# adwardlee/RenderIH

Measured on AMD Instinct MI355X. Metric: images/sec fwd+bwd @256x256 two-hand, higher is better.
Workload: dtype f32; 1 GPU; BASELINE configs[1]: batch=64/GPU 256x256 ResNet50 + cross-hand attention decoder, fwd + loss + bwd + Adam step, dropout 0.05, fp32; global_batch=64, parallelism=dp1, hipgraph=True, backward_stages=1, weight_gradients_on_side_stream=False, grad_allreduce=none (1 rank), optimizer=renderih_amd.optim.Adam (rih_adam_multi, one launch), flash_attention=True, one_kernel_attention_rih_fused_attn=False

## Files before the change

### include/renderih_amd.h

```cpp
#ifndef RENDERIH_AMD_H
#define RENDERIH_AMD_H

#include <stdint.h>

#ifdef __cplusplus
extern "C" {
#endif

#define RIH_OK 0
#define RIH_EINVAL (-1)

typedef struct rih_gemm_desc {
    const float* A;
    const float* B;
    float* C;
    const float* bias;
    const float* R;
    int32_t M, N, K;
    int32_t lda, ldb, ldc, ldr;
    int32_t a_mode, b_mode;
    int32_t nb1, nb2;
    int64_t sA1, sA2, sB1, sB2, sC1, sC2;
    int32_t splitk;
    int32_t kchunk;
// ... 46 lines not shown
    float* dst;
    float* db;
    int32_t S, Mp, M, N, Cin, taps, CinValid, accumulate;
    int32_t CinPitch;
    int32_t reserved;
} rih_reduce_desc;
int rih_splitk_reduce_multi(const rih_reduce_desc* descs, int n, void* stream);
int rih_splitk_reduce_bias_batched(const float* P, int S, int Mp, int M, int N, float* dst, int Cin, int taps,
                                   int CinValid, int accumulate, float* db, int nb, int64_t sP, int64_t sDst,
                                   int64_t sDb, void* stream);

int rih_bn_stats_from_blocks(const float* part, int T, int C, int rows, int rows_per_block, float eps, float momentum,
                             float* mean, float* invstd, float* running_mean, float* running_var, void* stream);

typedef struct rih_conv3_desc {
    const float* x;
    const void* w_h2;
    float* y;
    float* stats;
    const float* amax_x;
    const float* amax_w;
    int32_t imgs, H, W, C, N, ldx, ldy, Kpad, relu;
    int32_t ldr;
    const float* r;
} rih_conv3_desc;
int rih_conv3x3_ok(const rih_conv3_desc* d);
int rih_conv3x3_stats_rows(const rih_conv3_desc* d);
int rih_conv3x3(const rih_conv3_desc* d, void* stream);
typedef struct rih_h2_desc {
    const float* w;
    void* dst;
    const float* amax;
    int32_t Cout, Cin, KH, KW, CinPad, for_dgrad, Kpad;
} rih_h2_desc;
int rih_h2_multi(const rih_h2_desc* descs, int n, void* stream);

typedef struct rih_panel_desc {
    const float* a;
    const void* w_h2;
    float* c;
    const float* r;
    float* stats;
    const float* amax_a;
    const float* amax_w;
    int32_t M, N, K, lda, ldc, ldr, relu;
} rih_panel_desc;
int rih_panel_ok(const rih_panel_desc* d);
int rih_panel_stats_rows(const rih_panel_desc* d);
int rih_panel(const rih_panel_desc* d, void* stream);
int rih_stem_ok(const rih_conv3_desc* d);
int rih_stem(const rih_conv3_desc* d, void* stream);
int rih_rows_ok(const rih_panel_desc* d);
int rih_rows_stats_rows(const rih_panel_desc* d);
int rih_rows(const rih_panel_desc* d, void* stream);
int rih_rows_tile(const rih_panel_desc* d, int* bm, int* bn);
int rih_rows_tiled(const rih_panel_desc* d, int bm, int bn, void* stream);

int rih_splitk_finish(const float* P, int S, int M, int N, float* C, int ldc, const float* bias, const float* R,
                      int ldr, float alpha, int relu, void* stream);

int rih_pack_conv_weight(const float* w, float* dst, int Cout, int Cin, int KH, int KW, int CinPad,
                         int for_dgrad, void* stream);
typedef struct rih_pack_desc {
    const float* w;
    float* dst;
    int32_t Cout, Cin, KH, KW, CinPad, mode, kh0, kw0, step, Th, Tw, reserved;
} rih_pack_desc;
int rih_pack_conv_weight_multi(const rih_pack_desc* descs, int n, void* stream);
int rih_pack_conv_weight_sub(const float* w, float* dst, int Cout, int Cin, int KH, int KW, int CinPad, int kh0,
                             int kw0, int step, int Th, int Tw, void* stream);

int rih_nchw_to_nhwc(const float* x, float* y, int N, int C, int H, int W, int Cpad, void* stream);
int rih_nhwc_to_nchw(const float* x, float* y, int N, int C, int H, int W, int ldx, void* stream);
int rih_maxpool3x3s2_fwd(const float* x, float* y, int8_t* arg, int N, int H, int W, int C, void* stream);
int rih_maxpool3x3s2_bwd(const float* dy, const int8_t* arg, float* dx, int N, int H, int W, int C, void* stream);
int rih_avgpool_fwd(const float* x, float* y, int N, int HW, int C, void* stream);
int rih_avgpool_bwd(const float* dy, float* dx, int N, int HW, int C, void* stream);
int rih_upsample2x_fwd(const float* x, float* y, int N, int H, int W, int C, void* stream);
int rih_upsample2x_bwd(const float* dy, float* dx, int N, int H, int W, int C, void* stream);
int rih_upsample_bilinear_fwd(const float* x, float* y, int N, int H, int W, int C, int factor, void* stream);
int rih_upsample_bilinear_bwd(const float* dy, float* dx, int N, int H, int W, int C, int factor, void* stream);
int rih_nearest_up_add_fwd(const float* x, const float* add, float* y, int N, int H, int W, int C, int factor,
                           void* stream);
int rih_nearest_up_bwd(const float* dy, float* dx, int N, int H, int W, int C, int factor, void* stream);

int64_t rih_bn_ws_floats(int rows, int C);
int rih_bn_stats(const float* x, int rows, int C, float eps, float momentum, float* mean, float* invstd,
                 float* running_mean, float* running_var, float* ws, void* stream);
int rih_bn_eval_stats(const float* running_mean, const float* running_var, int C, float eps, float* mean,
                      float* invstd, void* stream);
int rih_bn_apply(const float* x, const float* mean, const float* invstd, const float* gamma, const float* beta,
                 const float* residual, float* y, int rows, int C, int relu, uint8_t* relu_mask, float* amax, void* stream);
int rih_bn_bwd(const float* dy, const float* x, const float* y, const float* mean, const float* invstd,
               const float* gamma, float* dx, float* dres, float* dgamma, float* dbeta, int rows, int C,
               int relu, int frozen_stats, float* ws, const uint8_t* relu_mask, float* amax_dx, void* stream);

int rih_layernorm_fwd(const float* x, const float* x2, const float* g, const float* b, float* y, float* mean,
                      float* rstd, int rows, int D, float eps, int relu, void* stream);
int rih_ln_nblk(int rows);
// ... 265 lines not shown
```

### renderih_amd/_lib.py

```python
import ctypes as C
import os

from . import _build

c_f = C.c_void_p
c_i = C.c_int
c_l = C.c_int64
c_u64 = C.c_uint64
c_fl = C.c_float


class GemmDesc(C.Structure):
    _fields_ = [('A', C.c_void_p), ('B', C.c_void_p), ('C', C.c_void_p), ('bias', C.c_void_p), ('R', C.c_void_p),
                ('M', C.c_int32), ('N', C.c_int32), ('K', C.c_int32),
                ('lda', C.c_int32), ('ldb', C.c_int32), ('ldc', C.c_int32), ('ldr', C.c_int32),
                ('a_mode', C.c_int32), ('b_mode', C.c_int32),
                ('nb1', C.c_int32), ('nb2', C.c_int32),
                ('sA1', C.c_int64), ('sA2', C.c_int64), ('sB1', C.c_int64), ('sB2', C.c_int64),
                ('sC1', C.c_int64), ('sC2', C.c_int64),
                ('splitk', C.c_int32), ('kchunk', C.c_int32), ('sCsplit', C.c_int64),
                ('alpha', C.c_float), ('relu', C.c_int32),
                ('H', C.c_int32), ('W', C.c_int32), ('Cin', C.c_int32), ('Ho', C.c_int32), ('Wo', C.c_int32),
                ('KH', C.c_int32), ('KW', C.c_int32), ('strideA', C.c_int32), ('upS', C.c_int32),
                ('padH', C.c_int32), ('padW', C.c_int32), ('tile', C.c_int32), ('engine', C.c_int32),
                ('cS', C.c_int32), ('cOH', C.c_int32), ('cOW', C.c_int32), ('cH', C.c_int32), ('cW', C.c_int32), ('ones_row', C.c_int32),
                ('reserved0', C.c_int32), ('sBias1', C.c_int64), ('sR1', C.c_int64), ('stats', C.c_void_p),
                ('drop_p', C.c_float), ('reserved1', C.c_int32), ('drop_seed', C.c_uint64), ('drop_seed_dev', C.c_void_p),
                ('amax_a', C.c_void_p), ('amax_b', C.c_void_p),
                ('a_seg', C.c_void_p * 3), ('lda_seg', C.c_int32 * 3), ('k_seg', C.c_int32 * 3)]


class ReduceDesc(C.Structure):
    _fields_ = [('P', C.c_void_p), ('dst', C.c_void_p), ('db', C.c_void_p)] + \
               [(n, C.c_int32) for n in ('S', 'Mp', 'M', 'N', 'Cin', 'taps', 'CinValid', 'accumulate', 'CinPitch', 'reserved')]


class Conv3Desc(C.Structure):
    _fields_ = [('x', C.c_void_p), ('w_h2', C.c_void_p), ('y', C.c_void_p), ('stats', C.c_void_p), ('amax_x', C.c_void_p),
                ('amax_w', C.c_void_p)] + \
               [(n, C.c_int32) for n in ('imgs', 'H', 'W', 'C', 'N', 'ldx', 'ldy', 'Kpad', 'relu', 'ldr')] + [('r', C.c_void_p)]


class PanelDesc(C.Structure):
    _fields_ = [('a', C.c_void_p), ('w_h2', C.c_void_p), ('c', C.c_void_p), ('r', C.c_void_p), ('stats', C.c_void_p),
                ('amax_a', C.c_void_p), ('amax_w', C.c_void_p)] + \
               [(n, C.c_int32) for n in ('M', 'N', 'K', 'lda', 'ldc', 'ldr', 'relu')]


class H2Desc(C.Structure):
    _fields_ = [('w', C.c_void_p), ('dst', C.c_void_p), ('amax', C.c_void_p)] + \
               [(n, C.c_int32) for n in ('Cout', 'Cin', 'KH', 'KW', 'CinPad', 'for_dgrad', 'Kpad')]


class AbsmaxDesc(C.Structure):
    _fields_ = [('x', C.c_void_p), ('out', C.c_void_p), ('n', C.c_int64)]


BOUND_FLOATS = 2048


class LnFinalDesc(C.Structure):
    _fields_ = [('ws', C.c_void_p), ('dg', C.c_void_p), ('db', C.c_void_p), ('D', C.c_int32), ('nblk', C.c_int32)]


class PackDesc(C.Structure):
    _fields_ = [('w', C.c_void_p), ('dst', C.c_void_p)] + \
               [(n, C.c_int32) for n in ('Cout', 'Cin', 'KH', 'KW', 'CinPad', 'mode', 'kh0', 'kw0', 'step', 'Th', 'Tw',
                                         'reserved')]


class HConvDesc(C.Structure):
    _fields_ = [('x', C.c_void_p), ('w', C.c_void_p), ('zero', C.c_void_p), ('bias', C.c_void_p),
                ('post_scale', C.c_void_p), ('post_shift', C.c_void_p), ('res', C.c_void_p), ('y', C.c_void_p)] + \
               [(n, C.c_int32) for n in ('N', 'H', 'W', 'Cin', 'Cout', 'KH', 'KW', 'stride', 'pad', 'Ho', 'Wo',
                                         'ldx', 'ldr', 'ldy', 'Kpad', 'relu', 'out_f32')]


class ManoModel(C.Structure):
    _fields_ = [('comps', C.c_void_p), ('hands_mean', C.c_void_p), ('shapedirs', C.c_void_p),
                ('posedirs', C.c_void_p), ('v_template', C.c_void_p), ('J_reg', C.c_void_p),
                ('weights', C.c_void_p), ('parent', C.c_int32 * 16)]


class MeshTopo(C.Structure):
# ... 220 lines not shown
```

### renderih_amd/csrc/rih_conv3.hip

```cpp
#include <hip/hip_runtime.h>
#include <stdint.h>
#include <stdlib.h>
#include "../../include/renderih_amd.h"
#include "rih_e2.h"

typedef float floatx16 __attribute__((ext_vector_type(16)));
typedef _Float16 f16x8 __attribute__((ext_vector_type(8)));

namespace {

constexpr int A_STAGE = 340 * 128;
constexpr int NT = 512;

struct C3Args {
    const float* x;
    const unsigned char* w;
    float* y;
    float* stats;
    const float* amax_x;
    const float* amax_w;
    int imgs, H, W, C, N, ldx, ldy, Kp, relu;
    int tiles_x, tiles_y, nblk;
    const float* r;
    int ldr;
// ... 204 lines not shown
                const int row = (lane >> 3) + 8 * q, c4 = (lane & 7) * 4;
                const int ty = (TW == 32) ? blk : 2 * blk + (row >> 4), tx = row & (TW - 1);
                float4 v = *reinterpret_cast<const float4*>(stg + row * SLD + c4);
                if (RES) {
                    const float4 rr = *reinterpret_cast<const float4*>(rpatch + ((long long)ty * p.W + tx) * p.ldr + j * 32 + c4);
                    v.x += rr.x; v.y += rr.y; v.z += rr.z; v.w += rr.w;
                }
                if (p.relu) { v.x = fmaxf(v.x, 0.f); v.y = fmaxf(v.y, 0.f); v.z = fmaxf(v.z, 0.f); v.w = fmaxf(v.w, 0.f); }
                *reinterpret_cast<float4*>(ypatch + ((long long)ty * p.W + tx) * p.ldy + j * 32 + c4) = v;
                if (STATS) RIH_E2_STATS_ADD(j, v)
            }
        }
    }
    if (STATS) {
        const long long rb = (((long long)img * p.tiles_y + ty_t) * p.tiles_x + tx_t) * WGM + wm;
#pragma unroll
        for (int j = 0; j < TN; ++j) {
            RIH_E2_STATS_MERGE(j, mean, m2)
            if ((lane >> 3) == 0) {
                const int nn = n0 + wn * (BN / WGN) + j * 32 + (lane & 7) * 4;
                *reinterpret_cast<float4*>(p.stats + (rb * 2 + 0) * p.N + nn) = mean;
                *reinterpret_cast<float4*>(p.stats + (rb * 2 + 1) * p.N + nn) = m2;
            }
        }
    }
}

struct H2WArgs {
    const float* w;
    unsigned char* dst;
    const float* amax;
    int N, K, Kp, for_dgrad;
    int Cout, Cin, KH, KW, CinPad;
};
__device__ __forceinline__ float h2w_fetch(const H2WArgs& a, int n, int k) {
    if (k >= a.K) return 0.f;
    if (!a.for_dgrad) {
        const int tap = k / a.CinPad, ci = k - tap * a.CinPad;
        return ci < a.Cin ? a.w[((long long)n * a.Cin + ci) * (a.KH * a.KW) + tap] : 0.f;
    }
    const int co = k % a.Cout, t = k / a.Cout;
    const int tw = t % a.KW, th = t / a.KW;
    const int kh = a.KH - 1 - th, kw = a.KW - 1 - tw;
    return n < a.Cin ? a.w[(((long long)co * a.Cin + n) * a.KH + kh) * a.KW + kw] : 0.f;
}
__device__ __forceinline__ void h2w_span(const H2WArgs& a, long long first, long long stride) {
    const int G = a.Kp / 8;
    const long long total = (long long)a.N * G;
    const float sc = e2_scale(a.amax);
    for (long long i = first; i < total; i += stride) {
        const int n = (int)(i / G), g = (int)(i - (long long)n * G);
        uint4 h, l;
        e2_split2h(h2w_fetch(a, n, 8 * g + 0), h2w_fetch(a, n, 8 * g + 1), sc, h.x, l.x);
        e2_split2h(h2w_fetch(a, n, 8 * g + 2), h2w_fetch(a, n, 8 * g + 3), sc, h.y, l.y);
        e2_split2h(h2w_fetch(a, n, 8 * g + 4), h2w_fetch(a, n, 8 * g + 5), sc, h.z, l.z);
        e2_split2h(h2w_fetch(a, n, 8 * g + 6), h2w_fetch(a, n, 8 * g + 7), sc, h.w, l.w);
        uint4* d = reinterpret_cast<uint4*>(a.dst + i * 32);
        d[0] = h;
        d[1] = l;
    }
}
constexpr int H2_PACK = 48;
struct H2Pack {
    H2WArgs d[H2_PACK];
    int first[H2_PACK + 1];
    int n;
};
static_assert(sizeof(H2Pack) <= 4096, "kernel argument limit");
__global__ __launch_bounds__(256) void h2_weight_multi_kernel(const H2Pack pk) {
    const int b = (int)blockIdx.x;
    int k = 0;
    while (k + 1 < pk.n && b >= pk.first[k + 1]) ++k;
    const int nb = pk.first[k + 1] - pk.first[k];
    h2w_span(pk.d[k], (long long)(b - pk.first[k]) * 256 + threadIdx.x, (long long)nb * 256);
}

int h2_args(H2WArgs& a, const rih_h2_desc& d) {
    if (!d.w || !d.dst || !d.amax || d.Cout < 1 || d.Cin < 1 || d.KH < 1 || d.KW < 1 || d.CinPad < d.Cin || d.Kpad < 32 ||
        d.Kpad % 32 != 0 || ((uintptr_t)d.dst % 16) != 0)
        return RIH_EINVAL;
    a.w = d.w; a.dst = (unsigned char*)d.dst; a.amax = d.amax; a.Kp = d.Kpad; a.for_dgrad = d.for_dgrad ? 1 : 0;
    a.Cout = d.Cout; a.Cin = d.Cin; a.KH = d.KH; a.KW = d.KW; a.CinPad = d.CinPad;
    if (!a.for_dgrad) { a.N = d.Cout; a.K = d.KH * d.KW * d.CinPad; }
    else { a.N = d.CinPad; a.K = d.KH * d.KW * d.Cout; }
    return a.Kp < a.K ? RIH_EINVAL : RIH_OK;
}


struct PanelArgs {
    const float* a;
    const unsigned char* w;
    float* c;
    const float* r;
    float* stats;
    const float* amax_a;
    const float* amax_w;
    int M, N, K, lda, ldc, ldr, relu;
    int nblk, mtiles;
};

template <int KT, int BN, bool STATS, bool RES>
__global__ __launch_bounds__(NT, 2) void panel_kernel(const PanelArgs p) {
    constexpr int K = 32 * KT;
    constexpr int BM = 8192 / K;
    constexpr int WGN = BN >= 128 ? 4 : 2, WGM = 8 / WGN;
    constexpr int TM = BM / WGM / 32, TN = BN / WGN / 32;
    static_assert(TM >= 1 && TN >= 1 && BN * K <= 16384, "tile shape");
    constexpr int ROWB = K * 4;
    constexpr int UPR = K / 4;
    constexpr int A_ST = BM * ROWB;
    constexpr int B_BYTES = BN * ROWB;
    constexpr int NPA = (BM * K / 4) / NT;
    constexpr int NPB = (BN * UPR) / NT;
    static_assert((BM * K / 4) % NT == 0 && (BN * UPR) % NT == 0 && 8 * 32 * 32 * 4 <= A_ST, "loader / staging geometry");
    __shared__ __attribute__((aligned(16))) unsigned char smem[B_BYTES + 2 * A_ST];
    unsigned char* const Bs = smem;
    unsigned char* const Abuf = smem + B_BYTES;
// ... 574 lines not shown
    rows_tile(d, bm, bn);
    return rih_rows_tiled(d, bm, bn, stream);
}

extern "C" int rih_stem_ok(const rih_conv3_desc* d) { return stem_ok(d) ? 1 : 0; }

extern "C" int rih_stem(const rih_conv3_desc* d, void* stream) {
    if (!stem_ok(d)) return RIH_EINVAL;
    RowsArgs a;
    a.a = d->x; a.w = (const unsigned char*)d->w_h2; a.c = d->y; a.r = nullptr; a.stats = d->stats;
    a.amax_a = d->amax_x; a.amax_w = d->amax_w;
    a.H = d->H; a.W = d->W; a.Ho = d->H / 2; a.Wo = d->W / 2;
    a.M = d->imgs * a.Ho * a.Wo; a.N = d->N; a.K = d->Kpad; a.lda = 4; a.ldc = d->ldy; a.ldr = 0; a.relu = d->relu ? 1 : 0;
    a.nblk = 1;
    a.mtiles = a.M / 256;
    hipStream_t s = (hipStream_t)stream;
    if (d->stats != nullptr) hipLaunchKernelGGL((rows_kernel<256, 64, true, false, true>), dim3((unsigned)a.mtiles), dim3(NT), 0, s, a);
    else hipLaunchKernelGGL((rows_kernel<256, 64, false, false, true>), dim3((unsigned)a.mtiles), dim3(NT), 0, s, a);
    return (int)hipGetLastError();
}

extern "C" int rih_h2_multi(const rih_h2_desc* descs, int n, void* stream) {
    if (n < 0 || (n > 0 && !descs)) return RIH_EINVAL;
    for (int i0 = 0; i0 < n; i0 += H2_PACK) {
        H2Pack pk;
        pk.n = (n - i0 < H2_PACK) ? n - i0 : H2_PACK;
        int total = 0;
        for (int i = 0; i < pk.n; ++i) {
            const int rc = h2_args(pk.d[i], descs[i0 + i]);
            if (rc != RIH_OK) return rc;
            const long long units = (long long)pk.d[i].N * (pk.d[i].Kp / 8);
            long long nb = (units + 255) / 256;
            if (nb > 512) nb = 512;
            pk.first[i] = total;
            total += (int)nb;
        }
        pk.first[pk.n] = total;
        hipLaunchKernelGGL(h2_weight_multi_kernel, dim3(total), dim3(256), 0, (hipStream_t)stream, pk);
    }
    return (int)hipGetLastError();
}
```

### renderih_amd/csrc/rih_gemm.hip

```cpp
#include <hip/hip_runtime.h>
#include <stdint.h>
#include <stdlib.h>
#include "../../include/renderih_amd.h"
#include "rih_hash.h"
#include "rih_e2.h"

typedef float floatx16 __attribute__((ext_vector_type(16)));
typedef __bf16 bf16x8 __attribute__((ext_vector_type(8)));
typedef __bf16 bf16x2 __attribute__((ext_vector_type(2)));
typedef _Float16 f16x8 __attribute__((ext_vector_type(8)));

namespace {

constexpr int BK = 32;

struct GemmArgs {
    const float* A;
    const float* B;
    float* C;
    const float* bias;
    const float* R;
    int M, N, K;
    int lda, ldb, ldc, ldr;
    int nb2, splitk, kchunk;
// ... 1071 lines not shown
    __shared__ float tile[8][33];
    const int tx = threadIdx.x & 31, ty = threadIdx.x >> 5;
    const int tilesN = (N + 31) / 32;
    const int m0 = (bx / tilesN) * 8, n0 = (bx % tilesN) * 32;
    {
        const int m = m0 + ty, n = n0 + tx;
        const bool ok = (m < M && n < N);
        const float* q = P + (ok ? (long long)m * N + n : 0);
        float a0 = 0.f, a1 = 0.f, a2 = 0.f, a3 = 0.f;
        int k = 0;
        for (; k + 3 < S; k += 4) {
            a0 += q[(long long)k * slab];
            a1 += q[(long long)(k + 1) * slab];
            a2 += q[(long long)(k + 2) * slab];
            a3 += q[(long long)(k + 3) * slab];
        }
        for (; k < S; ++k) a0 += q[(long long)k * slab];
        tile[ty][tx] = ok ? (a0 + a1) + (a2 + a3) : 0.f;
    }
    __syncthreads();
    {
        const int m = m0 + (threadIdx.x & 7), n = n0 + (threadIdx.x >> 3);
        if (m < M && n < N) {
            const int tap = m / Cin, ci = m - tap * Cin;
            if (ci < CinValid) {
                const long long o = ((long long)n * pitch + ci) * taps + tap;
                const float v = tile[threadIdx.x & 7][threadIdx.x >> 3];
                dst[o] = accumulate ? dst[o] + v : v;
            }
        }
    }
}

__global__ __launch_bounds__(256) void splitk_reduce_fused_kernel(const float* __restrict__ P, int S, int Mp, int M, int N,
                                                                  float* __restrict__ dst, int Cin, int taps, int CinValid,
                                                                  int accumulate, float* __restrict__ db, int ntiles,
                                                                  long long sP, long long sDst, long long sDb) {
    P += blockIdx.y * sP;
    dst += blockIdx.y * sDst;
    if (db != nullptr) db += blockIdx.y * sDb;
    splitk_reduce_block(P, S, Mp, M, N, dst, Cin, taps, CinValid, accumulate, db, ntiles, (int)blockIdx.x);
}

constexpr int REDUCE_PACK = 56;
struct ReducePack {
    rih_reduce_desc d[REDUCE_PACK];
    int first[REDUCE_PACK + 1];
    int ntiles[REDUCE_PACK];
    int n;
};
static_assert(sizeof(ReducePack) <= 4096, "kernel argument limit");
__global__ __launch_bounds__(256) void splitk_reduce_multi_kernel(const ReducePack pk) {
    const int b = (int)blockIdx.x;
    int i = 0;
    while (i + 1 < pk.n && b >= pk.first[i + 1]) ++i;
    const rih_reduce_desc& d = pk.d[i];
    splitk_reduce_block(d.P, d.S, d.Mp, d.M, d.N, d.dst, d.Cin, d.taps, d.CinValid, d.accumulate, d.db, pk.ntiles[i],
                        b - pk.first[i], d.CinPitch);
}

__global__ void splitk_finish_kernel(const float* __restrict__ P, int S, int M, int N, float* __restrict__ C, int ldc,
                                     const float* __restrict__ bias, const float* __restrict__ R, int ldr, float alpha,
                                     int relu) {
    const long long total = (long long)M * N;
    for (long long i = (long long)blockIdx.x * blockDim.x + threadIdx.x; i < total;
         i += (long long)gridDim.x * blockDim.x) {
        const int m = (int)(i / N), n = (int)(i - (long long)m * N);
        float s = 0.f;
        for (int k = 0; k < S; ++k) s += P[(long long)k * total + i];
        s *= alpha;
        if (bias != nullptr) s += bias[n];
        if (R != nullptr) s += R[(long long)m * ldr + n];
        if (relu) s = fmaxf(s, 0.f);
        C[(long long)m * ldc + n] = s;
    }
}

__global__ void pack_conv_weight_kernel(const float* __restrict__ w, float* __restrict__ dst, int Cout, int Cin,
                                        int KH, int KW, int CinPad, int for_dgrad) {
    const long long total = (long long)KH * KW * CinPad * Cout;
    for (long long i = (long long)blockIdx.x * blockDim.x + threadIdx.x; i < total;
         i += (long long)gridDim.x * blockDim.x) {
        int co, ci, tap;
        if (!for_dgrad) {
            co = (int)(i % Cout);
            const long long t = i / Cout;
            ci = (int)(t % CinPad);
            tap = (int)(t / CinPad);
        } else {
            ci = (int)(i % CinPad);
            const long long t = i / CinPad;
            co = (int)(t % Cout);
            tap = KH * KW - 1 - (int)(t / Cout);
        }
        float v = 0.f;
        if (ci < Cin) v = w[((long long)co * Cin + ci) * (KH * KW) + tap];
        dst[i] = v;
    }
}

__global__ void pack_conv_weight_sub_kernel(const float* __restrict__ w, float* __restrict__ dst, int Cout, int Cin,
                                            int KH, int KW, int CinPad, int kh0, int kw0, int step, int Th, int Tw) {
    const long long total = (long long)Th * Tw * Cout * CinPad;
    for (long long i = (long long)blockIdx.x * blockDim.x + threadIdx.x; i < total;
         i += (long long)gridDim.x * blockDim.x) {
        const int ci = (int)(i % CinPad);
        long long t = i / CinPad;
        const int co = (int)(t % Cout);
        t /= Cout;
        const int tw = (int)(t % Tw), th = (int)(t / Tw);
        const int kh = kh0 + step * (Th - 1 - th), kw = kw0 + step * (Tw - 1 - tw);
        dst[i] = (ci < Cin) ? w[(((long long)co * Cin + ci) * KH + kh) * KW + kw] : 0.f;
    }
}
constexpr int PACK_PACK = 56;
struct PackPack {
    rih_pack_desc d[PACK_PACK];
    int first[PACK_PACK + 1];
    int n;
};
static_assert(sizeof(PackPack) <= 4096, "kernel argument limit");
__global__ __launch_bounds__(256) void pack_conv_weight_multi_kernel(const PackPack pk) {
    const int b = (int)blockIdx.x;
    int k = 0;
    while (k + 1 < pk.n && b >= pk.first[k + 1]) ++k;
    const rih_pack_desc& d = pk.d[k];
    const int nb = pk.first[k + 1] - pk.first[k];
    const int taps = d.KH * d.KW;
    const long long total = (d.mode == 0) ? (long long)taps * d.CinPad * d.Cout : (long long)d.Th * d.Tw * d.Cout * d.CinPad;
    for (long long i = (long long)(b - pk.first[k]) * 256 + threadIdx.x; i < total; i += (long long)nb * 256) {
        float v = 0.f;
        if (d.mode == 0) {
            const int co = (int)(i % d.Cout);
            const long long t = i / d.Cout;
            const int ci = (int)(t % d.CinPad), tap = (int)(t / d.CinPad);
            if (ci < d.Cin) v = d.w[((long long)co * d.Cin + ci) * taps + tap];
        } else {
            const int ci = (int)(i % d.CinPad);
            long long t = i / d.CinPad;
            const int co = (int)(t % d.Cout);
            t /= d.Cout;
            const int tw = (int)(t % d.Tw), th = (int)(t / d.Tw);
            const int kh = d.kh0 + d.step * (d.Th - 1 - th), kw = d.kw0 + d.step * (d.Tw - 1 - tw);
            if (ci < d.Cin) v = d.w[(((long long)co * d.Cin + ci) * d.KH + kh) * d.KW + kw];
        }
        d.dst[i] = v;
    }
}

}

extern "C" int rih_pack_conv_weight_multi(const rih_pack_desc* descs, int n, void* stream) {
    if (n < 0 || (n > 0 && !descs)) return RIH_EINVAL;
    for (int i = 0; i < n; ++i) {
        const rih_pack_desc& d = descs[i];
        if (!d.w || !d.dst || d.Cout < 1 || d.Cin < 1 || d.KH < 1 || d.KW < 1 || d.CinPad < d.Cin || (d.mode != 0 && d.mode != 1))
            return RIH_EINVAL;
        if (d.mode == 1 && (d.step < 1 || d.Th < 1 || d.Tw < 1 || d.kh0 < 0 || d.kw0 < 0 ||
                            d.kh0 + d.step * (d.Th - 1) >= d.KH || d.kw0 + d.step * (d.Tw - 1) >= d.KW))
            return RIH_EINVAL;
    }
    for (int base = 0; base < n; base += PACK_PACK) {
        PackPack pk;
        pk.n = (n - base < PACK_PACK) ? n - base : PACK_PACK;
        int total = 0;
        for (int i = 0; i < pk.n; ++i) {
            const rih_pack_desc& d = descs[base + i];
            const long long el = (d.mode == 0) ? (long long)d.KH * d.KW * d.CinPad * d.Cout : (long long)d.Th * d.Tw * d.Cout * d.CinPad;
            long long nb = (el + 4095) / 4096;
            if (nb > 1024) nb = 1024;
            pk.d[i] = d;
            pk.first[i] = total;
            total += (int)nb;
        }
        pk.first[pk.n] = total;
        hipLaunchKernelGGL(pack_conv_weight_multi_kernel, dim3(total), dim3(256), 0, (hipStream_t)stream, pk);
    }
    return (int)hipGetLastError();
}
extern "C" int rih_pack_conv_weight_sub(const float* w, float* dst, int Cout, int Cin, int KH, int KW, int CinPad,
                                        int kh0, int kw0, int step, int Th, int Tw, void* stream) {
    if (!w || !dst || Cout < 1 || Cin < 1 || KH < 1 || KW < 1 || CinPad < Cin || step < 1 || Th < 1 || Tw < 1 ||
        kh0 < 0 || kw0 < 0 || kh0 + step * (Th - 1) >= KH || kw0 + step * (Tw - 1) >= KW)
        return RIH_EINVAL;
    const long long total = (long long)Th * Tw * Cout * CinPad;
    const int blocks = (int)((total + 255) / 256 < 4096 ? (total + 255) / 256 : 4096);
    hipLaunchKernelGGL(pack_conv_weight_sub_kernel, dim3(blocks), dim3(256), 0, (hipStream_t)stream, w, dst, Cout, Cin,
                       KH, KW, CinPad, kh0, kw0, step, Th, Tw);
    return (int)hipGetLastError();
}



struct PreparedGemm {
    GemmArgs a;
    int gx, gz, tile, a_mode, b_mode, plain, engine;
};

static int gemm_impl(const rih_gemm_desc* d, void* stream, int* stats_rows, PreparedGemm* prep = nullptr, int* engine_out = nullptr) {
    if (!d || !d->A || !d->B || !d->C) return RIH_EINVAL;
    if (d->M <= 0 || d->N <= 0 || d->K < 0) return RIH_EINVAL;
    if (d->splitk < 1 || d->nb1 < 1 || d->nb2 < 1) return RIH_EINVAL;
    if (d->splitk > 1 && (d->kchunk <= 0 || d->kchunk % BK != 0)) return RIH_EINVAL;
    if (d->Cin <= 0 || d->KH <= 0 || d->KW <= 0 || d->Ho <= 0 || d->Wo <= 0 || d->upS < 1 || d->strideA < 1)
// ... 233 lines not shown
        case 0 * 8 + 4 + 1: hipLaunchKernelGGL((gemm_split_multi_kernel<128, 128, 1, 0, true>), grid, block, 0, s, t); break;
        case 0 * 8 + 4 + 0: hipLaunchKernelGGL((gemm_split_multi_kernel<128, 128, 1, 0, false>), grid, block, 0, s, t); break;
        case 64 + 2 * 8 + 4 + 1: hipLaunchKernelGGL((gemm_split_multi_kernel<64, 64, 1, 0, true, 2>), grid, block, 0, s, t); break;
        case 64 + 2 * 8 + 4 + 0: hipLaunchKernelGGL((gemm_split_multi_kernel<64, 64, 1, 0, false, 2>), grid, block, 0, s, t); break;
        case 64 + 0 * 8 + 4 + 1: hipLaunchKernelGGL((gemm_split_multi_kernel<128, 128, 1, 0, true, 2>), grid, block, 0, s, t); break;
        case 64 + 0 * 8 + 4 + 0: hipLaunchKernelGGL((gemm_split_multi_kernel<128, 128, 1, 0, false, 2>), grid, block, 0, s, t); break;
        case 64 + 1 * 8 + 4 + 1: hipLaunchKernelGGL((gemm_split_multi_kernel<128, 64, 1, 0, true, 2>), grid, block, 0, s, t); break;
        case 64 + 1 * 8 + 4 + 0: hipLaunchKernelGGL((gemm_split_multi_kernel<128, 64, 1, 0, false, 2>), grid, block, 0, s, t); break;
        default: return RIH_EINVAL;
    }
    return (int)hipGetLastError();
}

extern "C" int rih_gemm_dropout_ok(const rih_gemm_desc* d) {
    if (!d) return 0;
    rih_gemm_desc c = *d;
    if (c.drop_p == 0.f) c.drop_p = 0.5f;
    c.stats = nullptr;
    int rows = 0;
    return gemm_impl(&c, nullptr, &rows) == 0 ? 1 : 0;
}

extern "C" int rih_gemm_stats_rows(const rih_gemm_desc* d) {
    int rows = 0;
    if (gemm_impl(d, nullptr, &rows) != 0) return 0;
    return rows;
}
extern "C" int rih_splitk_reduce_bias_batched(const float* P, int S, int Mp, int M, int N, float* dst, int Cin, int taps,
                                              int CinValid, int accumulate, float* db, int nb, int64_t sP, int64_t sDst,
                                              int64_t sDb, void* stream) {
    if (!P || !dst || S < 1 || M < 1 || Mp < M || N < 1 || Cin < 1 || taps < 1 || CinValid < 1) return RIH_EINVAL;
    if (db && Mp < M + 1) return RIH_EINVAL;
    if (nb < 1 || nb > 65535) return RIH_EINVAL;
    const long long tiles = (long long)((M + 7) / 8) * ((N + 31) / 32);
    const long long blocks = tiles + (db ? (N + 255) / 256 : 0);
    if (blocks > 0x7fffffffLL) return RIH_EINVAL;
    hipLaunchKernelGGL(splitk_reduce_fused_kernel, dim3((unsigned)blocks, (unsigned)nb), dim3(256), 0, (hipStream_t)stream,
                       P, S, Mp, M, N, dst, Cin, taps, CinValid, accumulate, db, (int)tiles, (long long)sP,
                       (long long)sDst, (long long)sDb);
    return (int)hipGetLastError();
}

extern "C" int rih_splitk_reduce_multi(const rih_reduce_desc* descs, int n, void* stream) {
    if (n < 0 || (n > 0 && !descs)) return RIH_EINVAL;
    for (int i = 0; i < n; ++i) {
        const rih_reduce_desc& d = descs[i];
        if (!d.P || !d.dst || d.S < 1 || d.M < 1 || d.Mp < d.M || d.N < 1 || d.Cin < 1 || d.taps < 1 || d.CinValid < 1)
            return RIH_EINVAL;
        if (d.db && d.Mp < d.M + 1) return RIH_EINVAL;
        if (d.CinPitch != 0 && d.CinPitch < d.CinValid) return RIH_EINVAL;
    }
    for (int base = 0; base < n; base += REDUCE_PACK) {
        ReducePack pk;
        pk.n = (n - base < REDUCE_PACK) ? n - base : REDUCE_PACK;
        long long total = 0;
        for (int i = 0; i < pk.n; ++i) {
            const rih_reduce_desc& d = descs[base + i];
            const long long tiles = (long long)((d.M + 7) / 8) * ((d.N + 31) / 32);
            pk.d[i] = d;
            pk.ntiles[i] = (int)tiles;
            pk.first[i] = (int)total;
            total += tiles + (d.db ? (d.N + 255) / 256 : 0);
            if (total > 0x7fffffffLL) return RIH_EINVAL;
        }
        pk.first[pk.n] = (int)total;
        hipLaunchKernelGGL(splitk_reduce_multi_kernel, dim3((unsigned)total), dim3(256), 0, (hipStream_t)stream, pk);
    }
    return (int)hipGetLastError();
}

extern "C" int rih_splitk_reduce_bias(const float* P, int S, int Mp, int M, int N, float* dst, int Cin, int taps,
                                      int CinValid, int accumulate, float* db, void* stream) {
    return rih_splitk_reduce_bias_batched(P, S, Mp, M, N, dst, Cin, taps, CinValid, accumulate, db, 1, 0, 0, 0, stream);
}

extern "C" int rih_splitk_reduce(float* P, int S, int M, int N, float* dst, int Cin, int taps, int CinValid,
                                 int accumulate, void* stream) {
    return rih_splitk_reduce_bias(P, S, M, M, N, dst, Cin, taps, CinValid, accumulate, nullptr, stream);
}

extern "C" int rih_splitk_finish(const float* P, int S, int M, int N, float* C, int ldc, const float* bias,
                                 const float* R, int ldr, float alpha, int relu, void* stream) {
    if (!P || !C || S < 1 || M < 1 || N < 1 || ldc < N || (R && ldr < N)) return RIH_EINVAL;
    const long long total = (long long)M * N;
    const int blocks = (int)((total + 255) / 256 < 8192 ? (total + 255) / 256 : 8192);
    hipLaunchKernelGGL(splitk_finish_kernel, dim3(blocks), dim3(256), 0, (hipStream_t)stream, P, S, M, N, C, ldc, bias, R,
                       ldr, alpha, relu);
    return (int)hipGetLastError();
}

extern "C" int rih_pack_conv_weight(const float* w, float* dst, int Cout, int Cin, int KH, int KW, int CinPad,
                                    int for_dgrad, void* stream) {
// ... 8 lines not shown
```

Measured before the change: 2095 images/sec.

## Add LDS-tiled transpose paths for weight packing, h2 conversion and split-K reduce

Adds shared-memory tiled kernels for three weight-side transforms. The h2 weight conversion, conv weight packing and split-K weight-gradient reduction now stage a block of weights or reduced rows in LDS before writing the transposed layout. This is meant to replace strided, uncoalesced global reads and writes. The split-K reduce also gains a deep path that reads S in parallel lanes and combines them with shuffles. Paths are chosen per descriptor through the reserved field, which adds complexity and may change summation order.

New measurement: 2122 images/sec (median of 6 runs). 1.3% higher.

```diff
diff --git a/include/renderih_amd.h b/include/renderih_amd.h
--- a/include/renderih_amd.h
+++ b/include/renderih_amd.h
@@ -102,6 +102,7 @@
     void* dst;
     const float* amax;
     int32_t Cout, Cin, KH, KW, CinPad, for_dgrad, Kpad;
+    int32_t reserved;
 } rih_h2_desc;
 int rih_h2_multi(const rih_h2_desc* descs, int n, void* stream);
 
@@ -134,7 +135,8 @@
 typedef struct rih_pack_desc {
     const float* w;
     float* dst;
-    int32_t Cout, Cin, KH, KW, CinPad, mode, kh0, kw0, step, Th, Tw, reserved;
+    int32_t Cout, Cin, KH, KW, CinPad, mode, kh0, kw0, step, Th, Tw;
+    int32_t reserved;
 } rih_pack_desc;
 int rih_pack_conv_weight_multi(const rih_pack_desc* descs, int n, void* stream);
 int rih_pack_conv_weight_sub(const float* w, float* dst, int Cout, int Cin, int KH, int KW, int CinPad, int kh0,
diff --git a/renderih_amd/_lib.py b/renderih_amd/_lib.py
--- a/renderih_amd/_lib.py
+++ b/renderih_amd/_lib.py
@@ -49,7 +49,7 @@
 
 class H2Desc(C.Structure):
     _fields_ = [('w', C.c_void_p), ('dst', C.c_void_p), ('amax', C.c_void_p)] + \
-               [(n, C.c_int32) for n in ('Cout', 'Cin', 'KH', 'KW', 'CinPad', 'for_dgrad', 'Kpad')]
+               [(n, C.c_int32) for n in ('Cout', 'Cin', 'KH', 'KW', 'CinPad', 'for_dgrad', 'Kpad', 'reserved')]
 
 
 class AbsmaxDesc(C.Structure):
diff --git a/renderih_amd/csrc/rih_conv3.hip b/renderih_amd/csrc/rih_conv3.hip
--- a/renderih_amd/csrc/rih_conv3.hip
+++ b/renderih_amd/csrc/rih_conv3.hip
@@ -260,6 +260,7 @@
     const float* amax;
     int N, K, Kp, for_dgrad;
     int Cout, Cin, KH, KW, CinPad;
+    int wide;
 };
 __device__ __forceinline__ float h2w_fetch(const H2WArgs& a, int n, int k) {
     if (k >= a.K) return 0.f;
@@ -288,6 +289,103 @@
         d[1] = l;
     }
 }
+constexpr int H2W_LDS = 4096;
+struct H2Tile { int cob, cib, lp, ok; };
+__host__ __device__ inline H2Tile h2w_tile(const H2WArgs& a) {
+    H2Tile t;
+    t.cob = t.cib = t.lp = t.ok = 0;
+    const long long taps = (long long)a.KH * a.KW;
+    if (taps > 127) return t;
+    if (!a.for_dgrad) {
+        if (a.CinPad % 8 == 0) t.cib = taps == 1 ? 64 : 32;
+        else if (a.CinPad * taps < H2W_LDS) t.cib = a.CinPad;
+        else return t;
+        t.lp = (t.cib * (int)taps) | 1;
+        if (t.lp > H2W_LDS) return t;
+        t.cob = H2W_LDS / t.lp > 64 ? 64 : H2W_LDS / t.lp;
+    } else {
+        if (a.Cout % 8 != 0) return t;
+        t.cob = 32;
+        t.cib = 127 / (int)taps > 64 ? 64 : 127 / (int)taps;
+        t.lp = (t.cib * (int)taps) | 1;
+    }
+    t.ok = 1;
+    return t;
+}
+inline long long h2w_wide_tiles(const H2WArgs& a, const H2Tile& t) {
+    return (long long)((a.Cout + t.cob - 1) / t.cob) * ((a.CinPad + t.cib - 1) / t.cib);
+}
+__device__ __forceinline__ void h2w_store(const H2WArgs& a, int n, int g, const float* v, float sc) {
+    uint4 h, l;
+    e2_split2h(v[0], v[1], sc, h.x, l.x);
+    e2_split2h(v[2], v[3], sc, h.y, l.y);
+    e2_split2h(v[4], v[5], sc, h.z, l.z);
+    e2_split2h(v[6], v[7], sc, h.w, l.w);
+    uint4* d = reinterpret_cast<uint4*>(a.dst + ((long long)n * (a.Kp / 8) + g) * 32);
+    d[0] = h;
+    d[1] = l;
+}
+__device__ __forceinline__ void h2w_wide_block(const H2WArgs& a, int bx) {
+    __shared__ float T[H2W_LDS];
+    const H2Tile t = h2w_tile(a);
+    const int taps = a.KH * a.KW, G = a.Kp / 8, lp = t.lp;
+    const int tilesCi = (a.CinPad + t.cib - 1) / t.cib;
+    const int co0 = (bx / tilesCi) * t.cob, ci0 = (bx % tilesCi) * t.cib;
+    const int cobv = a.Cout - co0 < t.cob ? a.Cout - co0 : t.cob;
+    const int cibv = a.CinPad - ci0 < t.cib ? a.CinPad - ci0 : t.cib;
+    const int span = cibv * taps;
+    const int live = a.Cin - ci0 < cibv ? (a.Cin - ci0 > 0 ? (a.Cin - ci0) * taps : 0) : span;
+#pragma unroll 4
+    for (int c = threadIdx.x >> 6; c < cobv; c += 4) {
+        const long long src = ((long long)(co0 + c) * a.Cin + ci0) * taps;
+        for (int e = threadIdx.x & 63; e < span; e += 64) T[c * lp + e] = e < live ? a.w[src + e] : 0.f;
+    }
+    __syncthreads();
+    const float sc = e2_scale(a.amax);
+    float v[8];
+    if (!a.for_dgrad && a.CinPad % 8 != 0) {
+        for (int i = threadIdx.x; i < cobv * G; i += 256) {
+            const int c = i / G, g = i - c * G;
+#pragma unroll
+            for (int j = 0; j < 8; ++j) {
+                const int k = 8 * g + j, tap = k / a.CinPad, ci = k - tap * a.CinPad;
+                v[j] = k < a.K ? T[c * lp + ci * taps + tap] : 0.f;
+            }
+            h2w_store(a, co0 + c, g, v, sc);
+        }
+        return;
+    }
+    const int g_pad = a.K / 8;
+    if (!a.for_dgrad) {
+        const int gpt = cibv / 8, per = taps * gpt;
+        for (int i = threadIdx.x; i < cobv * per; i += 256) {
+            const int c = i / per, r = i - c * per;
+            const int tap = r / gpt, q = r - tap * gpt;
+#pragma unroll
+            for (int j = 0; j < 8; ++j) v[j] = T[c * lp + (8 * q + j) * taps + tap];
+            h2w_store(a, co0 + c, (tap * a.CinPad + ci0) / 8 + q, v, sc);
+        }
+        if (ci0 != 0) return;
+#pragma unroll
+        for (int j = 0; j < 8; ++j) v[j] = 0.f;
+        for (int i = threadIdx.x; i < cobv * (G - g_pad); i += 256)
+            h2w_store(a, co0 + i / (G - g_pad), g_pad + i % (G - g_pad), v, sc);
+    } else {
+        const int gpc = cobv / 8, per = taps * gpc;
+        for (int i = threadIdx.x; i < cibv * per; i += 256) {
+            const int cl = i / per, r = i - cl * per;
+            const int tt = r / gpc, q = r - tt * gpc;
+#pragma unroll
+            for (int j = 0; j < 8; ++j) v[j] = T[(8 * q + j) * lp + cl * taps + (taps - 1 - tt)];
+            h2w_store(a, ci0 + cl, (tt * a.Cout + co0) / 8 + q, v, sc);
+        }
+        if (co0 != 0) return;
+#pragma unroll
+        for (int j = 0; j < 8; ++j) v[j] = 0.f;
+        for (int i = threadIdx.x; i < cibv * (G - g_pad); i += 256)
+            h2w_store(a, ci0 + i / (G - g_pad), g_pad + i % (G - g_pad), v, sc);
+    }
+}
 constexpr int H2_PACK = 48;
 struct H2Pack {
     H2WArgs d[H2_PACK];
@@ -300,7 +398,8 @@
     int k = 0;
     while (k + 1 < pk.n && b >= pk.first[k + 1]) ++k;
     const int nb = pk.first[k + 1] - pk.first[k];
-    h2w_span(pk.d[k], (long long)(b - pk.first[k]) * 256 + threadIdx.x, (long long)nb * 256);
+    if (pk.d[k].wide) h2w_wide_block(pk.d[k], b - pk.first[k]);
+    else h2w_span(pk.d[k], (long long)(b - pk.first[k]) * 256 + threadIdx.x, (long long)nb * 256);
 }
 
 int h2_args(H2WArgs& a, const rih_h2_desc& d) {
@@ -311,6 +410,7 @@
     a.Cout = d.Cout; a.Cin = d.Cin; a.KH = d.KH; a.KW = d.KW; a.CinPad = d.CinPad;
     if (!a.for_dgrad) { a.N = d.Cout; a.K = d.KH * d.KW * d.CinPad; }
     else { a.N = d.CinPad; a.K = d.KH * d.KW * d.Cout; }
+    a.wide = (d.reserved == 0 && h2w_tile(a).ok) ? 1 : 0;
     return a.Kp < a.K ? RIH_EINVAL : RIH_OK;
 }
 
@@ -951,6 +1051,8 @@
             const long long units = (long long)pk.d[i].N * (pk.d[i].Kp / 8);
             long long nb = (units + 255) / 256;
             if (nb > 512) nb = 512;
+            if (pk.d[i].wide) nb = h2w_wide_tiles(pk.d[i], h2w_tile(pk.d[i]));
+            if (total + nb > 0x7fffffffLL) return RIH_EINVAL;
             pk.first[i] = total;
             total += (int)nb;
         }
diff --git a/renderih_amd/csrc/rih_gemm.hip b/renderih_amd/csrc/rih_gemm.hip
--- a/renderih_amd/csrc/rih_gemm.hip
+++ b/renderih_amd/csrc/rih_gemm.hip
@@ -1127,14 +1127,191 @@
     }
 }
 
+constexpr int RW_NT = 32;
+constexpr int RW_ROWS = 96;
+constexpr int RW_LP = RW_ROWS + 1;
+__host__ __device__ inline int reduce_wide_ci(int taps) {
+    if (taps == 1) return 64;
+    return taps > 64 ? 1 : 64 / taps;
+}
+#define RIH_RW_ADD(A, V) { A.x += V.x; A.y += V.y; A.z += V.z; A.w += V.w; }
+#define RIH_RW_LD(Q, K) (*reinterpret_cast<const float4*>((Q) + (long long)(K) * slab))
+#define RIH_RW_FIN(R, A0, A1, A2, A3)                                                                                  \
+    { R.x = (A0.x + A1.x) + (A2.x + A3.x); R.y = (A0.y + A1.y) + (A2.y + A3.y);                                        \
+      R.z = (A0.z + A1.z) + (A2.z + A3.z); R.w = (A0.w + A1.w) + (A2.w + A3.w); }
+__device__ __forceinline__ float4 reduce_wide_row(const float* __restrict__ q, int S, long long slab) {
+    const float4 z = make_float4(0.f, 0.f, 0.f, 0.f);
+    float4 a0 = z, a1 = z, a2 = z, a3 = z;
+    int k = 0;
+    for (; k + 7 < S; k += 8) {
+        const float4 v0 = RIH_RW_LD(q, k), v1 = RIH_RW_LD(q, k + 1), v2 = RIH_RW_LD(q, k + 2), v3 = RIH_RW_LD(q, k + 3);
+        const float4 v4 = RIH_RW_LD(q, k + 4), v5 = RIH_RW_LD(q, k + 5), v6 = RIH_RW_LD(q, k + 6), v7 = RIH_RW_LD(q, k + 7);
+        RIH_RW_ADD(a0, v0) RIH_RW_ADD(a1, v1) RIH_RW_ADD(a2, v2) RIH_RW_ADD(a3, v3)
+        RIH_RW_ADD(a0, v4) RIH_RW_ADD(a1, v5) RIH_RW_ADD(a2, v6) RIH_RW_ADD(a3, v7)
+    }
+    for (; k + 3 < S; k += 4) {
+        const float4 v0 = RIH_RW_LD(q, k), v1 = RIH_RW_LD(q, k + 1), v2 = RIH_RW_LD(q, k + 2), v3 = RIH_RW_LD(q, k + 3);
+        RIH_RW_ADD(a0, v0) RIH_RW_ADD(a1, v1) RIH_RW_ADD(a2, v2) RIH_RW_ADD(a3, v3)
+    }
+    for (; k < S; ++k) { const float4 v = RIH_RW_LD(q, k); RIH_RW_ADD(a0, v) }
+    float4 r;
+    RIH_RW_FIN(r, a0, a1, a2, a3)
+    return r;
+}
+__device__ __forceinline__ void reduce_wide_row2(const float* __restrict__ qa, const float* __restrict__ qb, int S,
+                                                 long long slab, float4& ra, float4& rb) {
+    const float4 z = make_float4(0.f, 0.f, 0.f, 0.f);
+    float4 a0 = z, a1 = z, a2 = z, a3 = z, b0 = z, b1 = z, b2 = z, b3 = z;
+    int k = 0;
+    for (; k + 3 < S; k += 4) {
+        const float4 v0 = RIH_RW_LD(qa, k), v1 = RIH_RW_LD(qa, k + 1), v2 = RIH_RW_LD(qa, k + 2), v3 = RIH_RW_LD(qa, k + 3);
+        const float4 w0 = RIH_RW_LD(qb, k), w1 = RIH_RW_LD(qb, k + 1), w2 = RIH_RW_LD(qb, k + 2), w3 = RIH_RW_LD(qb, k + 3);
+        RIH_RW_ADD(a0, v0) RIH_RW_ADD(a1, v1) RIH_RW_ADD(a2, v2) RIH_RW_ADD(a3, v3)
+        RIH_RW_ADD(b0, w0) RIH_RW_ADD(b1, w1) RIH_RW_ADD(b2, w2) RIH_RW_ADD(b3, w3)
+    }
+    const int t = S - k;
+    if (t > 0) {
+        const float4 v0 = RIH_RW_LD(qa, k), w0 = RIH_RW_LD(qb, k);
+        const float4 v1 = RIH_RW_LD(qa, t > 1 ? k + 1 : k), w1 = RIH_RW_LD(qb, t > 1 ? k + 1 : k);
+        const float4 v2 = RIH_RW_LD(qa, t > 2 ? k + 2 : k), w2 = RIH_RW_LD(qb, t > 2 ? k + 2 : k);
+        RIH_RW_ADD(a0, v0) RIH_RW_ADD(b0, w0)
+        if (t > 1) { RIH_RW_ADD(a0, v1) RIH_RW_ADD(b0, w1) }
+        if (t > 2) { RIH_RW_ADD(a0, v2) RIH_RW_ADD(b0, w2) }
+    }
+    RIH_RW_FIN(ra, a0, a1, a2, a3)
+    RIH_RW_FIN(rb, b0, b1, b2, b3)
+}
+__device__ __forceinline__ void splitk_reduce_wide_block(const float* __restrict__ P, int S, int Mp, int M, int N,
+                                                         float* __restrict__ dst, int Cin, int taps, int CinValid,
+                                                         int accumulate, float* __restrict__ db, int ntiles, int bx,
+                                                         int CinPitch) {
+    if (bx >= ntiles) {
+        splitk_reduce_block(P, S, Mp, M, N, dst, Cin, taps, CinValid, accumulate, db, 0, bx - ntiles, CinPitch);
+        return;
+    }
+    __shared__ float wtile[RW_NT * RW_LP];
+    const int pitch = CinPitch > 0 ? CinPitch : CinValid;
+    const long long slab = (long long)Mp * N;
+    const int cr = reduce_wide_ci(taps);
+    const int tilesN = (N + RW_NT - 1) / RW_NT;
+    const int c0 = (bx / tilesN) * cr, n0 = (bx % tilesN) * RW_NT;
+    const int crv = CinValid - c0 < cr ? CinValid - c0 : cr;
+    const int rows = crv * taps;
+    {
+        const int nq = threadIdx.x & 7, n = n0 + 4 * nq;
+        if (n < N) {
+            float* t = wtile + 4 * nq * RW_LP;
+            for (int e = threadIdx.x >> 3; e < rows; e += 64) {
+                const int cj = e / taps, tap = e - cj * taps;
+                const float* qa = P + ((long long)tap * Cin + c0 + cj) * N + n;
+                float4 ra, rb;
+                if (e + 32 < rows) {
+                    const int cj2 = (e + 32) / taps, tap2 = e + 32 - cj2 * taps;
+                    reduce_wide_row2(qa, P + ((long long)tap2 * Cin + c0 + cj2) * N + n, S, slab, ra, rb);
+                    t[e + 32] = rb.x; t[RW_LP + e + 32] = rb.y; t[2 * RW_LP + e + 32] = rb.z; t[3 * RW_LP + e + 32] = rb.w;
+                } else {
+                    ra = reduce_wide_row(qa, S, slab);
+                }
+                t[e] = ra.x; t[RW_LP + e] = ra.y; t[2 * RW_LP + e] = ra.z; t[3 * RW_LP + e] = ra.w;
+            }
+        }
+    }
+    __syncthreads();
+    const int total = RW_NT * rows;
+    for (int i = threadIdx.x; i < total; i += 256) {
+        const int nl = i / rows, e = i - nl * rows;
+        if (n0 + nl < N) {
+            const long long o = ((long long)(n0 + nl) * pitch + c0) * taps + e;
+            const float v = wtile[nl * RW_LP + e];
+            dst[o] = accumulate ? dst[o] + v : v;
+        }
+    }
+}
+constexpr int RW_DEEP = 32;
+__device__ __forceinline__ float4 reduce_shfl_add(const float4& a, int mask) {
+    float4 r;
+    r.x = a.x + __shfl_xor(a.x, mask, 64); r.y = a.y + __shfl_xor(a.y, mask, 64);
+    r.z = a.z + __shfl_xor(a.z, mask, 64); r.w = a.w + __shfl_xor(a.w, mask, 64);
+    return r;
+}
+__device__ __forceinline__ void splitk_reduce_deep_block(const float* __restrict__ P, int S, int Mp, int M, int N,
+                                                         float* __restrict__ dst, int Cin, int taps, int CinValid,
+                                                         int accumulate, float* __restrict__ db, int ntiles, int bx,
+                                                         int CinPitch) {
+    if (bx >= ntiles) {
+        splitk_reduce_block(P, S, Mp, M, N, dst, Cin, taps, CinValid, accumulate, db, 0, bx - ntiles, CinPitch);
+        return;
+    }
+    __shared__ float dtile[8][33];
+    const int pitch = CinPitch > 0 ? CinPitch : CinValid;
+    const long long slab = (long long)Mp * N;
+    const int nq = threadIdx.x & 7, j = (threadIdx.x >> 3) & 3, rl = threadIdx.x >> 5;
+    const int tilesN = (N + 31) / 32;
+    const int m0 = (bx / tilesN) * 8, n0 = (bx % tilesN) * 32;
+    {
+        const int m = m0 + rl, n = n0 + 4 * nq;
+        const bool ok = (m < M && n < N);
+        const float* q = P + (ok ? (long long)m * N + n : 0);
+        const int S4 = S & ~3;
+        float4 a = make_float4(0.f, 0.f, 0.f, 0.f);
+        int k = j;
+        for (; k + 28 < S4; k += 32) {
+            const float4 v0 = RIH_RW_LD(q, k), v1 = RIH_RW_LD(q, k + 4), v2 = RIH_RW_LD(q, k + 8), v3 = RIH_RW_LD(q, k + 12);
+            const float4 v4 = RIH_RW_LD(q, k + 16), v5 = RIH_RW_LD(q, k + 20), v6 = RIH_RW_LD(q, k + 24), v7 = RIH_RW_LD(q, k + 28);
+            RIH_RW_ADD(a, v0) RIH_RW_ADD(a, v1) RIH_RW_ADD(a, v2) RIH_RW_ADD(a, v3)
+            RIH_RW_ADD(a, v4) RIH_RW_ADD(a, v5) RIH_RW_ADD(a, v6) RIH_RW_ADD(a, v7)
+        }
+        for (; k < S4; k += 4) { const float4 v = RIH_RW_LD(q, k); RIH_RW_ADD(a, v) }
+        if (j == 0)
+            for (k = S4; k < S; ++k) { const float4 v = RIH_RW_LD(q, k); RIH_RW_ADD(a, v) }
+        const float4 x = reduce_shfl_add(a, 8);
+        const float4 y = reduce_shfl_add(x, 16);
+        if (j == 0) {
+            dtile[rl][4 * nq] = ok ? y.x : 0.f; dtile[rl][4 * nq + 1] = ok ? y.y : 0.f;
+            dtile[rl][4 * nq + 2] = ok ? y.z : 0.f; dtile[rl][4 * nq + 3] = ok ? y.w : 0.f;
+        }
+    }
+    __syncthreads();
+    {
+        const int m = m0 + (threadIdx.x & 7), n = n0 + (threadIdx.x >> 3);
+        if (m < M && n < N) {
+            const int tap = m / Cin, ci = m - tap * Cin;
+            if (ci < CinValid) {
+                const long long o = ((long long)n * pitch + ci) * taps + tap;
+                const float v = dtile[threadIdx.x & 7][threadIdx.x >> 3];
+                dst[o] = accumulate ? dst[o] + v : v;
+            }
+        }
+    }
+}
+#undef RIH_RW_ADD
+#undef RIH_RW_LD
+#undef RIH_RW_FIN
+__device__ __forceinline__ void splitk_reduce_any(int path, const float* __restrict__ P, int S, int Mp, int M, int N,
+                                                  float* __restrict__ dst, int Cin, int taps, int CinValid, int accumulate,
+                                                  float* __restrict__ db, int ntiles, int bx, int CinPitch) {
+    if (path == 1) splitk_reduce_wide_block(P, S, Mp, M, N, dst, Cin, taps, CinValid, accumulate, db, ntiles, bx, CinPitch);
+    else if (path == 2) splitk_reduce_deep_block(P, S, Mp, M, N, dst, Cin, taps, CinValid, accumulate, db, ntiles, bx, CinPitch);
+    else splitk_reduce_block(P, S, Mp, M, N, dst, Cin, taps, CinValid, accumulate, db, ntiles, bx, CinPitch);
+}
+inline int reduce_path(const float* P, int S, int M, int N, int Cin, int taps, int CinValid) {
+    if (N % 4 != 0 || ((uintptr_t)P % 16) != 0 || taps > RW_ROWS || CinValid > Cin || (long long)taps * Cin != M) return 0;
+    return S >= RW_DEEP ? 2 : 1;
+}
+inline long long reduce_tiles(int path, int M, int N, int taps, int CinValid) {
+    if (path != 1) return (long long)((M + 7) / 8) * ((N + 31) / 32);
+    const int cr = reduce_wide_ci(taps);
+    return (long long)((CinValid + cr - 1) / cr) * ((N + RW_NT - 1) / RW_NT);
+}
+
 __global__ __launch_bounds__(256) void splitk_reduce_fused_kernel(const float* __restrict__ P, int S, int Mp, int M, int N,
                                                                   float* __restrict__ dst, int Cin, int taps, int CinValid,
                                                                   int accumulate, float* __restrict__ db, int ntiles,
-                                                                  long long sP, long long sDst, long long sDb) {
+                                                                  long long sP, long long sDst, long long sDb, int path) {
     P += blockIdx.y * sP;
     dst += blockIdx.y * sDst;
     if (db != nullptr) db += blockIdx.y * sDb;
-    splitk_reduce_block(P, S, Mp, M, N, dst, Cin, taps, CinValid, accumulate, db, ntiles, (int)blockIdx.x);
+    splitk_reduce_any(path, P, S, Mp, M, N, dst, Cin, taps, CinValid, accumulate, db, ntiles, (int)blockIdx.x, 0);
 }
 
 constexpr int REDUCE_PACK = 56;
@@ -1150,8 +1327,8 @@
     int i = 0;
     while (i + 1 < pk.n && b >= pk.first[i + 1]) ++i;
     const rih_reduce_desc& d = pk.d[i];
-    splitk_reduce_block(d.P, d.S, d.Mp, d.M, d.N, d.dst, d.Cin, d.taps, d.CinValid, d.accumulate, d.db, pk.ntiles[i],
-                        b - pk.first[i], d.CinPitch);
+    splitk_reduce_any(d.reserved, d.P, d.S, d.Mp, d.M, d.N, d.dst, d.Cin, d.taps, d.CinValid, d.accumulate, d.db, pk.ntiles[i],
+                      b - pk.first[i], d.CinPitch);
 }
 
 __global__ void splitk_finish_kernel(const float* __restrict__ P, int S, int M, int N, float* __restrict__ C, int ldc,
@@ -1215,11 +1392,67 @@
     int n;
 };
 static_assert(sizeof(PackPack) <= 4096, "kernel argument limit");
+constexpr int PW_TAPS = 63;
+constexpr int PW_LDS = 4096;
+struct PackTile { int cob, cib, lp; };
+__host__ __device__ inline PackTile pack_wide_tile(int taps, int mode) {
+    PackTile t;
+    if (mode == 0) {
+        t.cob = 64;
+        t.cib = 63 / taps;
+    } else {
+        t.cib = 64;
+        t.cob = PW_LDS / (64 * taps + 1) > 64 ? 64 : PW_LDS / (64 * taps + 1);
+    }
+    t.lp = (t.cib * taps) | 1;
+    return t;
+}
+__device__ __forceinline__ void pack_wide_block(const rih_pack_desc& d, int bx) {
+    __shared__ float ptile[PW_LDS];
+    const int taps = d.KH * d.KW;
+    const PackTile pt = pack_wide_tile(taps, d.mode);
+    const int tilesCi = (d.CinPad + pt.cib - 1) / pt.cib;
+    const int co0 = (bx / tilesCi) * pt.cob, ci0 = (bx % tilesCi) * pt.cib;
+    const int cobv = d.Cout - co0 < pt.cob ? d.Cout - co0 : pt.cob;
+    const int cibv = d.CinPad - ci0 < pt.cib ? d.CinPad - ci0 : pt.cib;
+    const int span = cibv * taps;
+    const int live = d.Cin - ci0 < cibv ? (d.Cin - ci0 > 0 ? (d.Cin - ci0) * taps : 0) : span;
+    const int wave = threadIdx.x >> 6, lane = threadIdx.x & 63;
+#pragma unroll 4
+    for (int c = wave; c < cobv; c += 4) {
+        const long long src = ((long long)(co0 + c) * d.Cin + ci0) * taps;
+        for (int e = lane; e < span; e += 64) ptile[c * pt.lp + e] = e < live ? d.w[src + e] : 0.f;
+    }
+    __syncthreads();
+    if (d.mode == 0) {
+        if (lane < cobv)
+            for (int tap = 0; tap < taps; ++tap)
+                for (int cj = wave; cj < cibv; cj += 4)
+                    d.dst[((long long)tap * d.CinPad + ci0 + cj) * d.Cout + co0 + lane] = ptile[lane * pt.lp + cj * taps + tap];
+    } else if (lane < cibv) {
+        for (int th = 0; th < d.Th; ++th)
+            for (int tw = 0; tw < d.Tw; ++tw) {
+                const int tap = (d.kh0 + d.step * (d.Th - 1 - th)) * d.KW + d.kw0 + d.step * (d.Tw - 1 - tw);
+                for (int c = wave; c < cobv; c += 4)
+                    d.dst[((long long)(th * d.Tw + tw) * d.Cout + co0 + c) * d.CinPad + ci0 + lane] =
+                        ptile[c * pt.lp + lane * taps + tap];
+            }
+    }
+}
+inline long long pack_wide_tiles(const rih_pack_desc& d) {
+    const PackTile pt = pack_wide_tile(d.KH * d.KW, d.mode);
+    return (long long)((d.Cout + pt.cob - 1) / pt.cob) * ((d.CinPad + pt.cib - 1) / pt.cib);
+}
+
 __global__ __launch_bounds__(256) void pack_conv_weight_multi_kernel(const PackPack pk) {
     const int b = (int)blockIdx.x;
     int k = 0;
     while (k + 1 < pk.n && b >= pk.first[k + 1]) ++k;
     const rih_pack_desc& d = pk.d[k];
+    if (d.reserved) {
+        pack_wide_block(d, b - pk.first[k]);
+        return;
+    }
     const int nb = pk.first[k + 1] - pk.first[k];
     const int taps = d.KH * d.KW;
     const long long total = (d.mode == 0) ? (long long)taps * d.CinPad * d.Cout : (long long)d.Th * d.Tw * d.Cout * d.CinPad;
@@ -1264,7 +1497,11 @@
             const long long el = (d.mode == 0) ? (long long)d.KH * d.KW * d.CinPad * d.Cout : (long long)d.Th * d.Tw * d.Cout * d.CinPad;
             long long nb = (el + 4095) / 4096;
             if (nb > 1024) nb = 1024;
+            const bool wide = d.reserved == 0 && (long long)d.KH * d.KW <= PW_TAPS;
+            if (wide) nb = pack_wide_tiles(d);
+            if (total + nb > 0x7fffffffLL) return RIH_EINVAL;
             pk.d[i] = d;
+            pk.d[i].reserved = wide ? 1 : 0;
             pk.first[i] = total;
             total += (int)nb;
         }
@@ -1564,12 +1801,13 @@
     if (!P || !dst || S < 1 || M < 1 || Mp < M || N < 1 || Cin < 1 || taps < 1 || CinValid < 1) return RIH_EINVAL;
     if (db && Mp < M + 1) return RIH_EINVAL;
     if (nb < 1 || nb > 65535) return RIH_EINVAL;
-    const long long tiles = (long long)((M + 7) / 8) * ((N + 31) / 32);
+    const int path = (nb == 1 || sP % 4 == 0) ? reduce_path(P, S, M, N, Cin, taps, CinValid) : 0;
+    const long long tiles = reduce_tiles(path, M, N, taps, CinValid);
     const long long blocks = tiles + (db ? (N + 255) / 256 : 0);
     if (blocks > 0x7fffffffLL) return RIH_EINVAL;
     hipLaunchKernelGGL(splitk_reduce_fused_kernel, dim3((unsigned)blocks, (unsigned)nb), dim3(256), 0, (hipStream_t)stream,
                        P, S, Mp, M, N, dst, Cin, taps, CinValid, accumulate, db, (int)tiles, (long long)sP,
-                       (long long)sDst, (long long)sDb);
+                       (long long)sDst, (long long)sDb, path);
     return (int)hipGetLastError();
 }
 
@@ -1588,8 +1826,10 @@
         long long total = 0;
         for (int i = 0; i < pk.n; ++i) {
             const rih_reduce_desc& d = descs[base + i];
-            const long long tiles = (long long)((d.M + 7) / 8) * ((d.N + 31) / 32);
+            const int path = d.reserved == 0 ? reduce_path(d.P, d.S, d.M, d.N, d.Cin, d.taps, d.CinValid) : 0;
+            const long long tiles = reduce_tiles(path, d.M, d.N, d.taps, d.CinValid);
             pk.d[i] = d;
+            pk.d[i].reserved = path;
             pk.ntiles[i] = (int)tiles;
             pk.first[i] = (int)total;
             total += tiles + (d.db ? (d.N + 255) / 256 : 0);
```
